# rhasspy/piper

Hardware: AMD Instinct MI355X
Metric: audio samples/sec (higher is better)
Workload: dtype f32; 1 GPU; BASELINE configs[1]: medium VITS voice (22050 Hz), 1 utterance(s) x 128 phoneme ids per step per GPU, scales 0.667/1.0/0.8; step = inferSeconds span: host ids in (pe_upload) + pe_run, engine draws both noise sites + int16 PCM to host (pe_fetch); parallelism=utterance-parallel x1, one process per GPU, RCCL weight broadcast

## Files before the change

piper_amd/csrc/engine.h:

```cpp
#pragma once
#include <cstdint>
#include <deque>
#include <list>
#include <map>
#include <string>
#include <unordered_map>
#include <vector>

#include "pe_rt.h"
#include "engine_buffers.h"
#include "kernels/params.h"
#include "policy.h"
#include "weights.h"

namespace pe {

struct PackedConv {
  float* wp = nullptr;
  float* wp16 = nullptr;
  float* wpb = nullptr;
  const float* wunscale = nullptr;
  float* wpg4 = nullptr;
  float* bias = nullptr;
  int rows = 0;
// ... 224 lines not shown
  const float* pack_ffn2(const WeightSet& ws, const std::string& wname);
  DevBuf<float> ffn_parts_;
  bool stage_a_ffn_fused() const;
  float* stage_a_enc_out() const;
  const float* w4_of(const float* w16) const { auto it = w4_of_.find(w16); return it == w4_of_.end() ? nullptr : it->second; }
  float* dp_proj16_ = nullptr;
  float* dp_pre16_ = nullptr;
  float* projpre4_ = nullptr; float* projpre_bias_ = nullptr; int projpre_split_ = 0;
  void colchain(const struct ColP& p, int B, int Lmax, double flops);
  bool conv1x1_col4(const float* w16, const float* bias, int rows, View in, View out, const int* lens, int B, int Lmax,
                    double flops, const float* bias2 = nullptr, long bias2_bs = 0, const float* w4direct = nullptr, int kin = 192,
                    long max_cols = 0);
  const float* pack4_conv_pad192(const WeightSet& ws, const std::string& wname, int in_rev, int out_rev);
  struct Rcl;
  void pack_gate4pre(const WeightSet& ws, const std::string& prefix, bool odd, Rcl& r);
  void gate_pre(const Rcl& r, View x0, View out, const int* lens, int Lmax, double cols, const float* b2);
  struct LnSecond { const float* w4 = nullptr; int split = 0; View out2{nullptr, 0, 0}; const float* bias2 = nullptr; long bias2_bs = 0; };
  void lngemm(View y, const float* g, const float* b, View x, const float* w16, const float* bias, int rows, View out,
              int T, double flops, const float* parts = nullptr, int nparts = 0, const float* pbias = nullptr,
              const LnSecond* second = nullptr);
  bool proj_pre_stacked() const;
  float* pack16_conv(const WeightSet& ws, const std::string& wname, int in_rev, int out_rev);
  int xcc_of_[64] = {0};
  int xcd_period_ = 0;
  void probe_xcds();
  static size_t col4_smem() { return ((size_t)4 * 196 + 4 * 192 * 4 + 32 + 64 * 4) * sizeof(float); }
  void issue_stage_a();
  void issue_stage_b();
  void issue_flow();
  void issue_window();
// ... 43 lines not shown
    float* proj16 = nullptr;
  };
  std::vector<CFlow> cflows_;
  float ea_m0_ = 0, ea_es0_ = 1;
  float *ea_dev_m_ = nullptr, *ea_dev_logs_ = nullptr;
 public:
  void arena_ready();
 private:
  struct Rcl {
    PackedConv pre, post;
    float *pre16 = nullptr, *post16 = nullptr;
    const float* pre4pad = nullptr;
    std::vector<PackedConv> in, rs;
    std::vector<const float*> rs4;
    const float* gpre4 = nullptr; const float* gpre_bias = nullptr; const float* gpre_tapb = nullptr;
    int in_off, out_off;
  };
  std::vector<Rcl> rcls_;
  PackedConv dec_pre_;
  struct UpStage {
    PackedConv up;
    int rate, ch;
    std::vector<std::vector<PackedConv>> rb;
    float* last_bias_sum = nullptr;
    struct HostConv { std::vector<float> w; int co = 0, ci = 0, k = 0, dil = 1; const float* bias = nullptr; };
    std::vector<std::vector<HostConv>> rb_host;
    void* mrf_phases = nullptr; float* mrf_w = nullptr;
    float* mrf_wsplit = nullptr; float* mrf_unscale = nullptr; int mrf_wsplit_floats = 0;
    int mrf_wfloats = 0, mrf_cp = 0, mrf_hx = 0;
    std::vector<struct MrfPhase> mrf_ph;
// ... 243 lines not shown
```

piper_amd/csrc/engine_issue.cpp:

```cpp
#include "engine_internal.h"

namespace pe {

bool Engine::stage_a_ffn_fused() const {
  double tsum = 0;
  for (int b = 0; b < B_; ++b) tsum += tlens_h_[b];
  const bool chain_q = pol_.chain16(tsum, false, H_, 96);
  bool f = pol_.ffn && chain_q && pol_.chain4((long)B_ * Tg_) && ffn_parts_ && (long)B_ * rup(Tg_, 4) <= LaunchPolicy::ffn_max_cols &&
           FC_ % 48 == 0 && FC_ / 48 <= 16 && w4_of(enc_proj16_);
  for (auto& e : enc_) f = f && e.f1p && e.f2p && w4_of(e.qkv16);
  return f;
}
bool Engine::proj_pre_stacked() const {
  double tsum = 0;
  for (int b = 0; b < B_; ++b) tsum += tlens_h_[b];
  return pol_.stack_pre && projpre4_ && projpre_split_ == enc_proj_.rows && dp_pre_.rows == 192 && H_ == 192 &&
         pol_.chain16(tsum, false, H_, 96) && pol_.chain4((long)B_ * Tg_);
}
float* Engine::stage_a_enc_out() const { return (stage_a_ffn_fused() && (enc_.size() & 1)) ? y_ : x_; }

void Engine::issue_stage_a() {
  const int B = B_, Ts = Ts_, T = Tg_;
  const long bsH = (long)H_ * Ts;
  auto V = [&](float* p, int ch) { return View{p, (long)ch * Ts, Ts}; };
// ... 279 lines not shown
    PE_LAUNCH_KB("regulate_kernel", 4.0 * (2.0 * C_ * cols_ids_ + 3.0 * C_ * fsum), launch::regulate(dim3((Fmax + 255) / 256, (C_ + 3) / 4, B), stream_, rp));
    if (zp_keep_)
      PE_HIP(hipMemcpyAsync(zp_keep_, zp_, (size_t)B * C_ * Fs * sizeof(float), hipMemcpyDeviceToDevice, stream_));
  }
  auto VF = [&](float* p, int ch) { return View{p, (long)ch * Fs, Fs}; };
  const View fh = VF(fh_, H_), facts = VF(facts_, H_), fskip = VF(fskip_, H_);
  const int half = C_ / 2;
  const bool chain = pol_.chain16(fsum, true, H_, half);
  auto rs_front_of = [&](size_t ri, bool front = true) {
    const Rcl& r = rcls_[ri];
    const int nl = (int)r.in.size();
    return chain && nl >= 1 && r.rs4[nl - 1] && r.rs[nl - 1].rows == H_ && H_ == 192 && half == 96 &&
           (front ? pol_.chain_rs_front((long)B * Fmax) : pol_.chain4_frames((long)B * Fmax)) && w4_of(r.post16) &&
           (ri + 1 >= rcls_.size() || (rcls_[ri + 1].pre.rows <= 192 && w4_of(rcls_[ri + 1].pre16)));
  };
  auto compose_pre_of = [&](size_t ri) {
    if (ri >= rcls_.size() || !pol_.compose_pre() || !rs_front_of(ri, false)) return false;
    const Rcl& r = rcls_[ri];
    return r.in.size() >= 2 && r.gpre4 && r.rs4[0] && r.rs[0].rows == 2 * H_ && w4_of(r.pre16) && r.pre.rows == H_ &&
           plan_conv(r.in[0], Fmax, EPI_GATE, stage_tiled_).form == CONV_GATE12;
  };
  for (size_t ri = 0; ri < rcls_.size(); ++ri) {
    Rcl& r = rcls_[ri];
    const View x0{zp_ + (long)r.in_off * Fs, (long)C_ * Fs, Fs};
    const View x1{zp_ + (long)r.out_off * Fs, (long)C_ * Fs, Fs};
    const bool compose_pre = compose_pre_of(ri);
    if (!(chain && ri > 0) && !compose_pre) {
      if (!(chain && r.pre4pad && conv1x1_col4(nullptr, r.pre.bias, r.pre.rows, x0, fh, lens_b_, B, Fmax, 2.0 * fsum * r.pre.macs_per_col,
                                               nullptr, 0, r.pre4pad, half, LaunchPolicy::col4_max_frames)))
        conv(r.pre, x0, fh, lens_b_, 1, Fmax, EPI_STORE);
    }
    const int nl = (int)r.in.size();
    const bool rs_front = rs_front_of(ri);
    for (int i = 0; i < nl; ++i) {
      const float* b2 = nspk_ > 1 ? cond_ + cond_off_wn_[ri] + (long)i * 2 * H_ : nullptr;
      if (compose_pre && i == 0) gate_pre(r, x0, facts, lens_b_, Fmax, fsum, b2);
      else conv(r.in[i], fh, facts, lens_b_, 1, Fmax, EPI_GATE, {.bias2 = b2, .bias2_bs = cond_bs_});
      if (rs_front && i == nl - 1) {
        fl += 2.0 * fsum * (r.in[i].macs_per_col + r.rs[i].macs_per_col);
        continue;
      }
      if (r.rs4[i] && pol_.chain4_frames((long)B * Fmax) && H_ == 192 && r.rs[i].rows <= 2 * H_) {
        ColP cp{};
        cp.in1 = facts.p; cp.in1_bs = facts.bs; cp.in1_cs = facts.cs; cp.K1 = H_;
        cp.w1 = r.rs4[i]; cp.b1 = r.rs[i].bias; cp.rows1 = r.rs[i].rows;
        cp.mode = 2; cp.first = i == 0 ? 1 : 0;
        cp.xcd = xcd_period_;
        cp.x1 = fh.p; cp.x1_bs = fh.bs; cp.x1_cs = fh.cs;
        cp.out = fskip.p; cp.out_bs = fskip.bs; cp.out_cs = fskip.cs;
        cp.lens = lens_b_;
        const bool hpre = compose_pre && i == 0;
        if (hpre) {
          cp.in0 = x0.p; cp.in0_bs = x0.bs; cp.in0_cs = x0.cs;
          cp.w2 = w4_of(r.pre16); cp.b2 = r.pre.bias; cp.rows2 = H_;
        }
        const int kh4 = kbegin(prof_level_ >= 2 ? krow("colchain4_kernel<false>") : 0,
                               2.0 * fsum * (r.rs[i].macs_per_col + (hpre ? r.pre.macs_per_col : 0)),
                               4.0 * (fsum * (H_ + 2.0 * cp.rows1) + (double)cp.rows1 * H_ + (hpre ? half * (fsum + H_) : 0)));
        launch::colchain4(dim3((Fmax + 3) / 4, B, (cp.rows1 + 191) / 192), col4_smem() + (hpre ? 4 * (96 + 4) * sizeof(float) : 0), stream_, cp);
        kend(kh4);
      } else {
        conv(r.rs[i], facts, fh, lens_b_, 1, Fmax, EPI_WNRS, {.out2 = fskip, .mode = i == 0 ? 1 : 0});
      }
      fl += 2.0 * fsum * (r.in[i].macs_per_col + r.rs[i].macs_per_col);
    }
    if (chain) {
      ColP cp{};
      cp.in1 = fskip.p; cp.in1_bs = fskip.bs; cp.in1_cs = fskip.cs; cp.K1 = H_;
      cp.w1 = r.post16; cp.b1 = r.post.bias; cp.rows1 = half;
      cp.mode = 1;
      cp.x1 = x1.p; cp.x1_bs = x1.bs; cp.x1_cs = x1.cs;
      if (ri + 1 < rcls_.size() && !compose_pre_of(ri + 1)) {
        const Rcl& nx = rcls_[ri + 1];
        if (nx.in_off != r.out_off) throw std::runtime_error("coupling layers do not alternate halves");
        cp.w2 = nx.pre16; cp.b2 = nx.pre.bias; cp.rows2 = H_;
        cp.out2 = fh.p; cp.o2_bs = fh.bs; cp.o2_cs = fh.cs;
      }
      cp.lens = lens_b_;
      if (rs_front) {
        cp.in0 = facts.p; cp.in0_bs = facts.bs; cp.in0_cs = facts.cs;
        cp.w0 = r.rs4[nl - 1]; cp.b0 = r.rs[nl - 1].bias; cp.first = nl == 1 ? 1 : 0;
      }
      colchain(cp, B, Fmax, 2.0 * fsum * (r.post.macs_per_col + (cp.w2 ? rcls_[ri + 1].pre.macs_per_col : 0) +
                                          (rs_front ? r.rs[nl - 1].macs_per_col : 0)));
    } else {
      conv(r.post, fskip, x1, lens_b_, 1, Fmax, EPI_SUBFROM);
    }
    fl += 2.0 * fsum * (r.pre.macs_per_col + r.post.macs_per_col);
  }
  prof_end(2, fl);

}

void Engine::issue_stage_b() {
  issue_flow();
  double fsum = 0;
  for (int b = 0; b < B_; ++b) fsum += frames_h_[b];
  issue_decoder(zp_, lens_b_, Fg_, fsum, false);
}
// ... 193 lines not shown
```

piper_amd/csrc/engine_launch.cpp:

```cpp
#include "engine_internal.h"

namespace pe {


static int tile_cfg_of(int cfg) { return cfg == CFG_C ? CFG_C : CFG_S; }
static int slab_halo(int xhalo) { return xhalo <= 64 ? 64 : 128; }
static size_t tile_smem(int nbuf, int BN, int halo) { return (size_t)nbuf * KC * ((BN + halo + 63) / 64 * 64) * sizeof(float); }
static size_t splitk_smem(int nw, int MT, int xw) { return std::max<size_t>((size_t)nw * KC * xw, (size_t)nw * MT * 16 * 64) * sizeof(float); }

ConvPlan Engine::plan_conv(const PackedConv& pc, int Lmax, int epi, bool stage_tiled) const {
  ConvPlan pl;
  const bool convt = epi == EPI_CONVT;
  const int ncols = pl.ncols = convt ? Lmax + 1 : Lmax;
  const int xhalo = (pc.ntaps - 1) * pc.dil, units = pc.nchunks * pc.ntaps;
  pl.blocks = tile_workgroups(CFG_BM[pc.cfg], CFG_BN[pc.cfg], ncols, pc.mtiles, B_);
  pl.halo = slab_halo(xhalo);
  const bool to_splitk = !stage_tiled && pol_.splitk(pl.blocks, xhalo, pc.Cin);
  const bool direct = pol_.one_tap_direct(pc.gate, convt, pc.ntaps, pc.Cin);
  pl.group_splitk = !stage_tiled && !convt && pol_.groupable(pc.gate, pc.up != 0, pl.blocks, xhalo, pc.Cin);
  pl.group_tiled = !pc.gate && pc.up == 0 && !convt && !to_splitk && !(matrix_bf3_ && pc.wpb) && !direct && xhalo <= 128;
  pl.group_cfg = tile_cfg_of(pc.cfg);
  if (to_splitk && epi == EPI_GATE &&
      pol_.gate_12col(pc.gate, pc.wpg4 != nullptr && pc.Cin == 192, pc.ntaps, pc.dil, tile_workgroups(32, 12, ncols, pc.split / 32, B_))) {
    pl.form = CONV_GATE12;
// ... 490 lines not shown
  cp.mode = 3;
  cp.xcd = xcd_period_;
  cp.res = bias2; cp.res_bs = bias2_bs;
  cp.out = out.p; cp.out_bs = out.bs; cp.out_cs = out.cs;
  cp.lens = lens;
  if (kt_on_ && out.p == qkv_ && rows == 3 * H_) { cp.kT = kT_; cp.vQ = vQ_; cp.kt_bs = (long)Ts_ * H_; kt_valid_ = true; }
  const double cols = lens == d_tlens_ ? cols_ids_ : cols_frames_;
  const int kh4 = kbegin(prof_level_ >= 2 ? krow("colchain4_kernel<false>") : 0, flops, 4.0 * (cols * (kin + rows) + (double)rows * kin));
  launch::colchain4(dim3((Lmax + 3) / 4, B, (rows + 191) / 192), col4_smem(), stream_, cp);
  kend(kh4);
  return true;
}

void Engine::colchain(const ColP& p, int B, int Lmax, double flops) {
  const double cols = p.lens == d_tlens_ ? cols_ids_ : cols_frames_;
  const double kbytes = 4.0 * (cols * (p.K1 + 2.0 * p.rows1 + (p.w2 ? p.rows2 : 0)) + (double)p.rows1 * p.K1 +
                               (p.w2 ? (double)p.rows2 * p.rows1 : 0.0));
  if ((p.mode == 1 ? pol_.chain4_frames((long)B * Lmax) : pol_.chain4((long)B * Lmax)) && p.K1 == 192 && (p.mode == 0 ? p.rows1 == 192 : (p.rows1 == 96 && (!p.w2 || p.rows2 <= 192)))) {
    const float* w1 = w4_of(p.w1);
    const float* w2 = p.w2 ? w4_of(p.w2) : nullptr;
    if (w1 && (!p.w2 || w2)) {
      ColP q = p;
      q.w1 = w1; q.w2 = w2;
      q.xcd = xcd_period_;
      const double kb0 = q.w0 ? 4.0 * (cols * 192.0 + 192.0 * 192.0) : 0.0;
      const int kh4 = kbegin(prof_level_ >= 2 ? krow(q.w0 ? "colchain4_kernel<true>" : "colchain4_kernel<false>") : 0, flops, kbytes + kb0);
      launch::colchain4(dim3((Lmax + 3) / 4, B), col4_smem(), stream_, q);
      kend(kh4);
      return;
    }
  }
  if (p.w0) throw std::runtime_error("internal: a res/skip conv in front of a chain that does not take the 4-column form");
  const int kh = kbegin(prof_level_ >= 2 ? krow("colchain_kernel<6>") : 0, flops, kbytes);
  const size_t smem = ((size_t)2 * 6 * 32 * 16 + 16 * 16) * sizeof(float);
  launch::colchain(dim3((Lmax + 15) / 16, B), smem, stream_, p);
  kend(kh);
}

int Engine::kbegin(int row, double flops, double bytes) {
  if (prof_level_ < 2) return -1;
  hipEvent_t a, b;
  if (ev_pool_.size() >= 2) {
    a = ev_pool_.back(); ev_pool_.pop_back();
    b = ev_pool_.back(); ev_pool_.pop_back();
  } else {
    PE_HIP(hipEventCreate(&a));
    PE_HIP(hipEventCreate(&b));
// ... 45 lines not shown
```

piper_amd/csrc/engine_pack.cpp:

```cpp
#include "engine_internal.h"
#include <cmath>

namespace pe {


float* Engine::dev_alloc(size_t nfloats, const float* src) {
  arena_off_ = (arena_off_ + 255) / 256 * 256;
  const size_t bytes = std::max<size_t>(nfloats, 1) * sizeof(float);
  if (arena_off_ + bytes > arena_bytes_) throw std::runtime_error("internal: packed weights exceed the arena bound");
  float* d = reinterpret_cast<float*>(arena_ + arena_off_);
  arena_off_ += bytes;
  if (src && nfloats && !skeleton_) PE_HIP(hipMemcpy(d, src, nfloats * sizeof(float), hipMemcpyHostToDevice));
  weight_bytes_ += nfloats * sizeof(float);
  return d;
}
float* Engine::dev_copy(const std::vector<float>& v) { return dev_alloc(v.size(), v.data()); }

float* Engine::dev_tensor(const WeightSet& ws, const std::string& name) {
  const HostTensor& t = ws.get(name);
  return dev_alloc((size_t)t.numel(), t.data.empty() ? nullptr : t.data.data());
}

size_t Engine::arena_bound(const WeightSet& ws) {
  size_t n = 0;
// ... 339 lines not shown
          bk += a * bp[c];
        }
        for (int i = 0; i < Ci; ++i)
          G[((((size_t)g * nt + k) * (Ci / 4) + i / 4) * 64 + lane) * 4 + (i & 3)] = (float)acc[i];
        tapb[(size_t)k * R + row] = (float)bk;
        bs += bk;
      }
      bsum[row] = (float)bs;
    }
  }
  r.gpre4 = dev_alloc(n4, skeleton_ ? nullptr : G.data());
  r.gpre_bias = dev_alloc((size_t)R, skeleton_ ? nullptr : bsum.data());
  r.gpre_tapb = dev_alloc((size_t)6 * R, skeleton_ ? nullptr : tapb.data());
}

DdsW Engine::load_dds(const WeightSet& ws, const std::string& p) {
  DdsW d;
  for (int i = 0; i < arch_[A_DDSLAYERS]; ++i) {
    const std::string s = std::to_string(i);
    d.dw_w.push_back(dev_tensor(ws, p + ".convs_sep." + s + ".weight"));
    d.dw_b.push_back(dev_tensor(ws, p + ".convs_sep." + s + ".bias"));
    d.c1x1.push_back(pack_conv(ws, p + ".convs_1x1." + s + ".weight", p + ".convs_1x1." + s + ".bias", 1, -1,
                               false, 0, 0));
    {
      const HostTensor& w1 = ws.get(p + ".convs_1x1." + s + ".weight");
      d.w16.push_back(pack16(w1.data, (int)w1.dims[0], (int)w1.dims[1]));
    }
    d.g1.push_back(dev_tensor(ws, p + ".norms_1." + s + ".gamma"));
    d.b1.push_back(dev_tensor(ws, p + ".norms_1." + s + ".beta"));
    d.g2.push_back(dev_tensor(ws, p + ".norms_2." + s + ".gamma"));
// ... 122 lines not shown
        r.in.push_back(pack_conv(ws, p + ".enc.in_layers." + s + ".weight", p + ".enc.in_layers." + s + ".bias",
                                 1, -1, true, 0, 0));
        r.rs.push_back(pack_conv(ws, p + ".enc.res_skip_layers." + s + ".weight",
                                 p + ".enc.res_skip_layers." + s + ".bias", 1, -1, false, 0, 0));
        {
          const HostTensor& wrs = ws.get(p + ".enc.res_skip_layers." + s + ".weight");
          r.rs4.push_back(wrs.dims.size() == 3 && wrs.dims[2] == 1 ? pack4(wrs.data, (int)wrs.dims[0], (int)wrs.dims[1]) : nullptr);
        }
        (void)wnk;
      }
      r.post = pack_conv(ws, p + ".post.weight", p + ".post.bias", 1, -1, false, 0, odd);
      r.pre16 = pack16_conv(ws, p + ".pre.weight", odd, 0);
      if (H_ == 192 && rcls_.empty()) r.pre4pad = pack4_conv_pad192(ws, p + ".pre.weight", odd, 0);
      r.post16 = pack16_conv(ws, p + ".post.weight", 0, odd);
      if (wnl >= 2) pack_gate4pre(ws, p, odd, r);
      rcls_.push_back(r);
      if (gin_) {
        const HostTensor& cw = ws.get(p + ".enc.cond_layer.weight");
        cond_wn_.push_back(CondW{dev_tensor(ws, p + ".enc.cond_layer.weight"), dev_tensor(ws, p + ".enc.cond_layer.bias"),
                                 (int)cw.dims[0]});
      }
    }
    if (flips & 1) throw std::runtime_error("odd number of flow layers is not supported");
  }

  dec_pre_ = pack_conv(ws, "dec.conv_pre.weight", "dec.conv_pre.bias", 1, -1, false, 0, 0);
  {
    const int nk = arch_[A_NRB], nd = arch_[A_NDIL];
    int ch = U_;
    for (int i = 0; i < arch_[A_NUPS]; ++i) {
// ... 224 lines not shown
```

piper_amd/csrc/kernels/col4.h:

```cpp
#pragma once
#include "dds.h"

namespace pe {

__device__ __forceinline__ int c4_tile(int bx, int nx, int P) { return pe_xcd_tile(bx, nx, P); }

constexpr int FFN_MAXS = 16;
constexpr int C4_H = 192, C4_NT = C4_H / 64;
template <int K>
struct Col4W {
  static constexpr int NQ = K / 16;
  static constexpr int KS = K + 4;
  f32x4 w[C4_NT][K / 16];
};
template <int K>
__device__ __forceinline__ void col_gemm4_fetch(Col4W<K>& W, const float* wp4, int nt, int wv, int lane) {
  constexpr int NQ = Col4W<K>::NQ, tile_floats = (K / 4) * 256;
#pragma unroll
  for (int m = 0; m < C4_NT; ++m) {
    const bool live = PE_UNIFORM(m < nt);
    const pe_rowsrc ws = pe_make_row_u(wp4 + (long)(live ? m : 0) * tile_floats, live ? tile_floats : 0);
#pragma unroll
    for (int q = 0; q < NQ; ++q) W.w[m][q] = pe_row_load4(ws, ((NQ * wv + q) * 64 + lane) * 4);
  }
// ... 59 lines not shown
}


template <bool FRONT>
__global__ __launch_bounds__(256) void colchain4_kernel(const int* lens, const float* in1, long in1_bs, int nx, int xcd, int mode,
                                                        int in1_cs, int K1r, int rows1, int first, int out_cs, ColP p) {
  PE_KTRACE(3);
  constexpr int NC = 4, NVT = 3, K1 = C4_H, K2 = C4_H / 2, KS1 = Col4W<K1>::KS, KS2 = Col4W<K2>::KS;
  PE_DYN_SMEM(float, sm);
  if constexpr (!FRONT) PE_STAMP(3, 0);
  p.lens = lens; p.xcd = xcd; p.mode = mode; p.in1 = in1; p.in1_bs = in1_bs; p.in1_cs = in1_cs; p.K1 = K1r; p.rows1 = rows1;
  p.first = first; p.out_cs = out_cs;
  const int b = blockIdx.y;
  int L = PE_UNIFORM(lens[b]);
  if constexpr (FRONT) PE_ENTRY_BATCH(L, p.res, p.res_bs, p.res_cs, p.gamma, p.beta, p.out, p.out_bs, p.x1, p.x1_bs, p.x1_cs, p.b1, p.w1,
                                      p.in0, p.in0_bs, p.in0_cs, p.w0, p.b0);
  else PE_ENTRY_BATCH(L, p.res, p.res_bs, p.res_cs, p.gamma, p.beta, p.out, p.out_bs, p.x1, p.x1_bs, p.x1_cs, p.b1, p.w1,
                      p.in0, p.in0_bs, p.in0_cs, p.w2, p.b2, p.kT, p.kt_bs, p.vQ);
  const int t0 = c4_tile(blockIdx.x, nx, p.xcd) * NC;
  if (t0 >= L) return;
  if constexpr (!FRONT) PE_STAMP(3, 1);
  float* YT = sm;
  float* P = YT + NC * KS1;
  float* red = P + 4 * C4_H * NC;
  const int tid = threadIdx.x, col = tid & 3, rl = tid >> 2, wv = PE_UNIFORM(tid >> 6), lane = tid & 63;
  const int t = t0 + col;
  const bool ok = t < L;
  const int part = p.mode >= 2 ? (int)blockIdx.z : 0, row0 = part * C4_H;
  const int rows_here = p.rows1 - row0 < C4_H ? p.rows1 - row0 : C4_H;
  Col4W<K1> gw0;
  Col4W<K1> gw;
  auto fetch_gw = [&]() { col_gemm4_fetch<K1>(gw, p.w1 + (long)part * C4_NT * (K1 / 4) * 256, (rows_here + 63) / 64, wv, lane); };
  const bool skip_part = p.mode == 2 && (p.rows1 <= C4_H || part == 1);
  const bool pre_part = !FRONT && p.mode == 2 && p.w2 && !skip_part;
  float* YTP = P + 4 * C4_H * NC + 32 + 64 * 4;
  Col4W<K2> gw2;
  float sk[NVT];
  if constexpr (FRONT) {
    const pe_rowsrc a0 = pe_make_row(p.in0 + (long)b * p.in0_bs, K1 * p.in0_cs);
    const pe_rowsrc s0 = pe_make_row(p.in1 + (long)b * p.in1_bs, p.first ? 0 : K1 * p.in1_cs);
    const pe_rowsrc b0d = pe_make_row(p.b0 ? p.b0 : p.w0, p.b0 ? K1 : 0);
    float av[NVT], b0v[NVT];
#pragma unroll
    for (int k = 0; k < NVT; ++k) {
      const int c = rl + 64 * k;
      av[k] = pe_row_load(a0, ok ? c * p.in0_cs + t : -1);
      sk[k] = pe_row_load(s0, ok ? c * p.in1_cs + t : -1);
      b0v[k] = pe_row_load(b0d, c);
    }
    PE_SCHED_FENCE();
    col_gemm4_fetch<K1>(gw0, p.w0, C4_NT, wv, lane);
// ... 34 lines not shown
    PE_SCHED_FENCE();
    if constexpr (!FRONT) fetch_gw();
    if (pre_part) col_gemm4_fetch<K2>(gw2, p.w2, C4_NT, wv, lane);
    if constexpr (!FRONT) PE_STAMP(3, 2);
#pragma unroll
    for (int k = 0; k < NVT; ++k) YT[col * KS1 + rl + 64 * k] = xin[k];
    if constexpr (!FRONT)
      if (pre_part) {
        YTP[col * KS2 + rl] = x0v[0];
        if (rl < K2 - 64) YTP[col * KS2 + rl + 64] = x0v[1];
      }
  }
  __syncthreads();
  if (pre_part) col_gemm4_run2<K1, K2>(gw, YT, gw2, YTP, P, wv, lane);
  else col_gemm4_run<K1>(gw, YT, P, wv, lane);
  const bool second = p.mode == 1 && p.w2;
  if (second) col_gemm4_fetch<K2>(gw2, p.w2, (p.rows2 + 63) / 64, wv, lane);
  __syncthreads();

  if (p.mode >= 2) {
    if (!ok) return;
    float* tp = (skip_part || p.mode == 3) ? p.out + (long)b * p.out_bs + (p.mode == 3 ? (long)row0 * p.out_cs : 0) : p.x1 + (long)b * p.x1_bs;
    const int tcs = (skip_part || p.mode == 3) ? p.out_cs : p.x1_cs;
#pragma unroll
    for (int k = 0; k < NVT; ++k) {
      const int c = rl + 64 * k;
      if (c < rows_here) {
        const float val = (col_gemm4_get(P, c, col) + b1v[k]) + ov[k];
        tp[(long)c * tcs + t] = val;
        if (p.mode == 3 && p.kT && part == 1) p.kT[(long)b * p.kt_bs + ((long)(c >> 2) * p.out_cs + t) * 4 + (c & 3)] = val;
        if (p.mode == 3 && p.vQ && part == 2) p.vQ[(long)b * p.kt_bs + ((long)(t >> 2) * C4_H + c) * 4 + (t & 3)] = val;
// ... 17 lines not shown
    float q = 0.f;
#pragma unroll
    for (int k = 0; k < NVT; ++k)
      if (rl + 64 * k < H) { const float d = v[k] - mean; q = fmaf(d, d, q); }
    const float rstd = 1.f / sqrtf(col_sum(q) / (float)H + 1e-5f);
    if (!ok) return;
    float* ob = p.out + (long)b * p.out_bs;
#pragma unroll
    for (int k = 0; k < NVT; ++k) {
      const int c = rl + 64 * k;
      if (c < H) ob[(long)c * p.out_cs + t] = (v[k] - mean) * rstd * gg[k] + bb[k];
    }
    return;
  }

  {
    float* xb = p.x1 + (long)b * p.x1_bs;
    float* YT2 = YT;
    const pe_rowsrc b2d = pe_make_row(second ? p.b2 : p.w1, (second && p.b2) ? p.rows2 : 0);
    float b2v[NVT];
#pragma unroll
    for (int k = 0; k < NVT; ++k) b2v[k] = pe_row_load(b2d, rl + 64 * k);
#pragma unroll
    for (int k = 0; k < NVT; ++k) {
      const int c = rl + 64 * k;
      if (c < K2) {
        const float xn = (ok && c < p.rows1) ? ov[k] - (col_gemm4_get(P, c, col) + b1v[k]) : 0.f;
        if (ok && c < p.rows1) xb[(long)c * p.x1_cs + t] = xn;
        YT2[col * KS2 + c] = xn;
      }
    }
    if (!second) return;
    __syncthreads();
    col_gemm4_run<K2>(gw2, YT2, P, wv, lane);
    __syncthreads();
    if (!ok) return;
    float* o2 = p.out2 + (long)b * p.o2_bs;
#pragma unroll
    for (int k = 0; k < NVT; ++k) {
      const int c = rl + 64 * k;
      if (c < p.rows2) o2[(long)c * p.o2_cs + t] = col_gemm4_get(P, c, col) + b2v[k];
    }
  }
}

__global__ __launch_bounds__(256) void lngemm4_kernel(const int* lens, int nx, int xcd, const float* in, long in_bs, int in_cs,
                                                      int rows, const float* parts, int nparts, LnGemmP p) {
  PE_KTRACE(7);
  constexpr int NC = 4, NVT = 3, H = C4_H, KS = Col4W<H>::KS;
  PE_DYN_SMEM(float, sm);
  p.lens = lens; p.xcd = xcd; p.in = in; p.in_bs = in_bs; p.in_cs = in_cs; p.rows = rows; p.parts = parts; p.nparts = nparts;
  const int b = blockIdx.y;
  int L = PE_UNIFORM(lens[b]);
  PE_ENTRY_BATCH(L, p.gamma, p.beta, p.bias, p.pbias, p.p_bs, p.w16);
  const int t0 = c4_tile(blockIdx.x, nx, p.xcd) * NC;
  if (t0 >= L) return;
  float* YT = sm;
  float* P = YT + NC * KS;
// ... 87 lines not shown
```

piper_amd/csrc/policy.cpp:

```cpp
#include "policy.h"

#include <cerrno>
#include <cstdio>
#include <cstdlib>
#include <cstring>
#include <mutex>
#include <stdexcept>
#include <string>

namespace pe {

static const LaunchPolicy::Knob kKnobs[] = {
    {"PIPER_HIP_MRF", &LaunchPolicy::mrf, 0, 2, "fused MRF stage kernel: 0 off (conv by conv), 1 by the measured policy (ResBlock2 stages always; ResBlock1 stages on 32 channels up to PIPER_HIP_MRF_MAXF frames per call), 2 wherever it applies"},
    {"PIPER_HIP_MRF_MAXF", &LaunchPolicy::mrf_maxf, 0, 1L << 40, "batch frames up to which a 32-channel ResBlock1 stage runs in the fused kernel (mode 1)"},
    {"PIPER_HIP_MRF_OU", &LaunchPolicy::mrf_ou, 0, 4, "force the output units per wave of mrf_kernel (1..4) instead of the cost model; ignored when the width does not fit"},
    {"PIPER_HIP_MRF_TAIL", &LaunchPolicy::mrf_tail, 0, 1, "generator tail inside the last stage's mrf_kernel (0: separate conv_post_kernel)"},
    {"PIPER_HIP_MRF_SPLIT", &LaunchPolicy::mrf_split, 0, 1, "matrix modes bf16x3 / f16x3: the fused MRF stage kernel on the 16-bit matrix pipe with split operands (mrf_split_kernel) wherever a fused stage applies; 0 = the f32 fused kernel below PIPER_HIP_BF3_MINF frames, conv by conv on the 16-bit pipe above"},
    {"PIPER_HIP_BF3_MINF", &LaunchPolicy::bf3_minf, 0, 1L << 40, "split matrix modes without a fused 16-bit stage kernel (bf16x6, or PIPER_HIP_MRF_SPLIT=0): batch frames from which the <= 64-channel MRF stages run conv by conv on the 16-bit pipe"},
    {"PIPER_HIP_SPLITK_MAX", &LaunchPolicy::splitk_max, 0, 1L << 40, "tile-workgroup count below which a conv goes to the split-K kernels (0: always the tiled kernel)"},
    {"PIPER_HIP_SPLITK16", &LaunchPolicy::splitk16, 0, 3, "16-column split-K form: 0 off, 1 gate convs, 2 + long-K plain convs, 3 everywhere"},
    {"PIPER_HIP_WIDE_SPLITK", &LaunchPolicy::wide_splitk, 0, 2, "12-wave split-K: 0 off, 1 WN gate conv, 2 always"},
    {"PIPER_HIP_TPB", &LaunchPolicy::tpb, 0, 64, "tiled kernel: column tiles walked by one workgroup (0 = 1)"},
    {"PIPER_HIP_GROUP_MRF", &LaunchPolicy::group_mrf, 0, 2, "sibling resblock convs of a wider small stage as grouped launches (one-utterance calls): 0 off, 2 without the K-concatenated last step"},
    {"PIPER_HIP_GROUP_MAXB", &LaunchPolicy::group_maxb, 0, 1L << 40, "64 x 64 tiles of one conv of a stage below which the grouped sibling launches of a single utterance take the split-K kernels (the tiled grouped launches from there on)"},
// ... 6 lines not shown
    {"PIPER_HIP_ATTN4", &LaunchPolicy::attn4, 0, 2, "attention + conv_o + norm_layers_1 on 4-query workgroups (attn4_kernel) in place of attno_kernel: 0 off, 1 for calls whose longest utterance has up to PIPER_HIP_ATTN4_MAXC ids, 2 wherever attno_kernel applies"},
    {"PIPER_HIP_ATTN4_MAXC", &LaunchPolicy::attn4_maxc, 0, 1L << 40, "ids of the longest utterance of a call up to which attention runs on 4-query workgroups"},
    {"PIPER_HIP_FUSE_DP", &LaunchPolicy::fuse_dp, 0, 1, "ConvFlow.pre / proj / spline fused into the DDSConv layer launches"},
    {"PIPER_HIP_SPEC", &LaunchPolicy::spec, 0, 1, "speculative stage-B sizing / whole utterance as one graph for <= 4 utterances per call"},
    {"PIPER_HIP_SPEC_EXPECT", &LaunchPolicy::spec_expect, 0, 1, "speculative graphs planned for the expected frame counts (0: for the bucket capacity)"},
    {"PIPER_HIP_PCM_ZC", &LaunchPolicy::pcm_zc, 0, 1, "PCM written straight into pinned host memory by pcm16_kernel (0: one copy per utterance behind the graph)"},
    {"PIPER_HIP_IDS_ZC", &LaunchPolicy::ids_zc, 0, 1, "phoneme ids, lengths and speaker ids read straight from the pinned host block by embed_kernel, up to 65536 padded ids per call (0: one host-to-device copy in front of the graph)"},
    {"PIPER_HIP_NO_GRAPH", &LaunchPolicy::no_graph, 0, 1, "launch kernels directly instead of replaying hipGraphs"},
    {"PIPER_HIP_GRAPHS", &LaunchPolicy::graphs, 1, 4096, "hipGraphs kept per engine (least recently used evicted one at a time)"},
    {"PIPER_HIP_CONVT_VEC", &LaunchPolicy::convt_vec, 0, 1, "polyphase up-conv: a lane's four accumulator rows leave as one 16-byte store (stride a multiple of 4) or two 8-byte stores (stride 2) of consecutive output samples; 0: one 4-byte store per phase"},
    {"PIPER_HIP_XCD", &LaunchPolicy::xcd, -1, 32, "XCDs the dispatch round-robins over, for the XCD-aware tile orders (-1 = probed at engine creation, 0 = tiles in workgroup order)"},
    {"PIPER_HIP_XCD_FFN", &LaunchPolicy::xcd_ffn, 0, 1, "ffn_kernel deals (column tile, slice) to the XCDs slice-major, so an XCD's L2 holds two slices' weights instead of all sixteen (0: blockIdx order)"},
    {"PIPER_HIP_STACK_PRE", &LaunchPolicy::stack_pre, 0, 1, "small calls of the 192-channel voices: enc_p.proj and dp.pre (both read the last LayerNorm's output) as one lngemm4_kernel launch over the stacked matrix (0: two launches)"},
    {"PIPER_HIP_CHAIN_RS", &LaunchPolicy::chain_rs, 0, 1, "small calls of the 192-channel voices: the last WN layer's res/skip conv (skip rows only) in front of the coupling layer's post + pre chain launch, colchain4_kernel<true> (0: a launch of its own)"},
    {"PIPER_HIP_GATE4", &LaunchPolicy::gate4, 0, 2, "short calls: the WN gate conv over 192 channels on 64-row x 12-column workgroups with the 4x4x1 MFMA (gate4_kernel) up to 640 workgroups: 0 off (16-column split-K form), 2 wherever the split-K route applies"},
    {"PIPER_HIP_WN_COMPOSE", &LaunchPolicy::wn_compose, 0, 3, "short calls of the 192-channel voices, where the coupling chain runs on colchain4_kernel and the gate conv on gate4_kernel: 1x1 convs of a coupling layer composed into their neighbours when the weights are packed: 0 off, 1 every composition that is built, 2 only pre into the first gate conv (gate4pre_kernel over the 96 channels of x0; the coupling layer's pre launch and the chain's pre GEMM go, the first res/skip launch also writes the hidden state's pre term), 3 only post into the skip convs (not built: the route of 0)"},
    {"PIPER_HIP_GATE_HALF", &LaunchPolicy::gate_half, 0, 1, "short one-utterance calls (up to 128 whole-group workgroups): the WN gate conv on half a 32-channel group per workgroup, six waves with the whole K range in flight, twice the workgroups (0: whole groups on twelve waves)"},
    {"PIPER_HIP_CONV1X1", &LaunchPolicy::conv1x1, 0, 1, "batched one-tap convs (q/k/v, WN res/skip, coupling pre/post, proj) through conv1x1_kernel, B operand straight from global memory (0: the tiled kernel)"},
    {"PIPER_HIP_WS_BUDGET_MB", &LaunchPolicy::ws_budget_mb, 0, 1048576, "MiB of device memory the workspace of one pipeline half may take (0: a third of the device's memory): capacities grow only inside it, a call that does not fit by itself is an error"},
    {"PIPER_HIP_ATTN_LONG", &LaunchPolicy::attn_long, 0, 1, "attention score slabs in global memory (attn_long_kernel) at every length, also in place of attno_kernel (tests): by default only utterances whose 32 x T slab does not fit LDS (more than ~830 ids) take that form"},
    {"PIPER_HIP_PROF_SITES", &LaunchPolicy::prof_sites, 0, 1, "level-2 profile rows of the tiled conv kernel per conv shape (tuning aid)"},
    {"PIPER_HIP_DEBUG_KEEP", &LaunchPolicy::debug_keep, 0, 1, "test hook: keep z_p for pe_debug_tensor"},
    {"PIPER_HIP_DEBUG_POISON", &LaunchPolicy::debug_poison, 0, 1, "test hook: activation workspaces are filled with NaN bit patterns when allocated (no kernel may read what the call did not write)"},
};

const LaunchPolicy::Knob* LaunchPolicy::knobs(int* n) {
  if (n) *n = (int)(sizeof(kKnobs) / sizeof(kKnobs[0]));
  return kKnobs;
}

void LaunchPolicy::read_env() {
// ... 45 lines not shown
```

piper_amd/csrc/policy.h:

```cpp
#pragma once
#include <cstddef>

namespace pe {

struct LaunchPolicy {
  long mrf = 1;
  long mrf_maxf = 1100;
  long mrf_ou = 0;
  long mrf_tail = 1;
  long mrf_split = 1;
  long bf3_minf = 1100;
  long splitk_max = 96;
  long splitk16 = 2;
  long wide_splitk = 1;
  long tpb = 0;
  long group_mrf = 1;
  long group_maxb = 160;
  long group_tiled = 1;
  long colchain = 1;
  long col4 = 1;
  long col4_maxc = 1024;
  long ffn = 1;
  long attno = 1;
  long attn4 = 1;
// ... 52 lines not shown
    return gate_half && gate && nchunks == 6 && ntaps <= 5 && 2 * workgroups_whole <= 256;
  }
  static constexpr long gate4_max_workgroups = 640;
  bool gate_12col(bool gate, bool packed4, int ntaps, int dil, long workgroups) const {
    return gate4 && gate && packed4 && ntaps <= 5 && dil == 1 && (gate4 == 2 || workgroups <= gate4_max_workgroups);
  }
  int tiles_per_workgroup() const { return tpb > 0 ? (int)tpb : 1; }
  bool chain16(double cols, bool frames, int k1, int half) const {
    return colchain && k1 == 192 && half == 96 && (colchain == 2 || cols <= (double)(frames ? colchain_max_frames : colchain_max_ids));
  }
  bool chain4(long cols, long limit = 0) const { return col4 && (col4 == 2 || cols <= (limit ? limit : col4_maxc)); }
  bool attn4_ids(long longest_utterance) const { return attn4 == 2 || (attn4 == 1 && longest_utterance <= attn4_maxc); }
  bool chain4_frames(long cols) const { return chain4(cols, col4_max_frames); }
  bool chain_rs_front(long cols) const { return chain_rs && chain4_frames(cols); }
  bool compose_pre() const { return wn_compose == 1 || wn_compose == 2; }
  bool mrf_build(int channels) const { return mrf != 0 && channels <= 64 && channels % 4 == 0; }
  bool mrf_stage(bool built, bool resblock1, int padded_channels, double frames, bool matrix_bf3, bool split_fused = false) const {
    if (mrf && built && split_fused) return mrf == 2 || !resblock1 || padded_channels == 32;
    return mrf && built && !(matrix_bf3 && mrf != 2 && frames >= (double)bf3_minf) &&
           (mrf == 2 || !resblock1 || (padded_channels == 32 && frames <= (double)mrf_maxf));
  }
  bool group_stage(int B, int nk, long blocks64, bool buffers_fit) const {
    return group_mrf && B == 1 && nk >= 2 && nk <= 3 && blocks64 < group_max_blocks64 && blocks64 < group_maxb && buffers_fit;
  }
  bool stage_all_tiled(int B, int nk, long blocks64) const {
    return group_mrf && group_tiled && B == 1 && nk >= 2 && nk <= 3 && blocks64 >= group_maxb;
  }
  bool group_sum() const { return group_mrf != 2; }
  bool group_stage_tiled(int nk, long tile_blocks, bool buffers_fit) const {
    return group_tiled && nk >= 2 && nk <= 3 && tile_blocks <= group_tiled_max_blocks && buffers_fit;
// ... 7 lines not shown
```

Measured before the change: 124.8 million samples/s.

## Compose coupling post 1x1 conv into WN skip convs and drop post GEMM

Precomputes post·skip weight products on the host so each WN res/skip layer writes the 96-row post contribution directly into the skip sum. The coupling chain launch then skips its 192->96 post GEMM through a new no-main path in colchain4_kernel. This removes one GEMM per coupling layer and shrinks the skip output from 192 to 96 rows. The cost is a new kernel branch and extra packed weights. The route only runs when wn_compose is 1 or 4, and the default value is not shown.

```diff
diff --git a/piper_amd/csrc/engine.h b/piper_amd/csrc/engine.h
--- a/piper_amd/csrc/engine.h
+++ b/piper_amd/csrc/engine.h
@@ -262,6 +262,7 @@
   const float* pack4_conv_pad192(const WeightSet& ws, const std::string& wname, int in_rev, int out_rev);
   struct Rcl;
   void pack_gate4pre(const WeightSet& ws, const std::string& prefix, bool odd, Rcl& r);
+  void pack_post4(const WeightSet& ws, const std::string& prefix, bool odd, Rcl& r);
   void gate_pre(const Rcl& r, View x0, View out, const int* lens, int Lmax, double cols, const float* b2);
   struct LnSecond { const float* w4 = nullptr; int split = 0; View out2{nullptr, 0, 0}; const float* bias2 = nullptr; long bias2_bs = 0; };
   void lngemm(View y, const float* g, const float* b, View x, const float* w16, const float* bias, int rows, View out,
@@ -335,6 +336,7 @@
     std::vector<PackedConv> in, rs;
     std::vector<const float*> rs4;
     const float* gpre4 = nullptr; const float* gpre_bias = nullptr; const float* gpre_tapb = nullptr;
+    std::vector<const float*> rsp4, rsp_bias;
     int in_off, out_off;
   };
   std::vector<Rcl> rcls_;
diff --git a/piper_amd/csrc/engine_issue.cpp b/piper_amd/csrc/engine_issue.cpp
--- a/piper_amd/csrc/engine_issue.cpp
+++ b/piper_amd/csrc/engine_issue.cpp
@@ -317,11 +317,20 @@
            (front ? pol_.chain_rs_front((long)B * Fmax) : pol_.chain4_frames((long)B * Fmax)) && w4_of(r.post16) &&
            (ri + 1 >= rcls_.size() || (rcls_[ri + 1].pre.rows <= 192 && w4_of(rcls_[ri + 1].pre16)));
   };
-  auto compose_pre_of = [&](size_t ri) {
-    if (ri >= rcls_.size() || !pol_.compose_pre() || !rs_front_of(ri, false)) return false;
+  auto compose_route_of = [&](size_t ri) {
+    if (ri >= rcls_.size() || !rs_front_of(ri, false)) return false;
     const Rcl& r = rcls_[ri];
     return r.in.size() >= 2 && r.gpre4 && r.rs4[0] && r.rs[0].rows == 2 * H_ && w4_of(r.pre16) && r.pre.rows == H_ &&
            plan_conv(r.in[0], Fmax, EPI_GATE, stage_tiled_).form == CONV_GATE12;
+  };
+  auto compose_pre_of = [&](size_t ri) { return pol_.compose_pre() && compose_route_of(ri); };
+  auto compose_post_of = [&](size_t ri) {
+    if (!pol_.compose_post() || !compose_route_of(ri)) return false;
+    const Rcl& r = rcls_[ri];
+    if (r.rsp4.size() != r.in.size()) return false;
+    for (size_t j = 0; j < r.rsp4.size(); ++j)
+      if (!r.rsp4[j] || !r.rsp_bias[j]) return false;
+    return true;
   };
   for (size_t ri = 0; ri < rcls_.size(); ++ri) {
     Rcl& r = rcls_[ri];
@@ -334,7 +343,7 @@
         conv(r.pre, x0, fh, lens_b_, 1, Fmax, EPI_STORE);
     }
     const int nl = (int)r.in.size();
-    const bool rs_front = rs_front_of(ri);
+    const bool rs_front = rs_front_of(ri), compose_post = compose_post_of(ri);
     for (int i = 0; i < nl; ++i) {
       const float* b2 = nspk_ > 1 ? cond_ + cond_off_wn_[ri] + (long)i * 2 * H_ : nullptr;
       if (compose_pre && i == 0) gate_pre(r, x0, facts, lens_b_, Fmax, fsum, b2);
@@ -347,6 +356,9 @@
         ColP cp{};
         cp.in1 = facts.p; cp.in1_bs = facts.bs; cp.in1_cs = facts.cs; cp.K1 = H_;
         cp.w1 = r.rs4[i]; cp.b1 = r.rs[i].bias; cp.rows1 = r.rs[i].rows;
+        if (compose_post) {
+          cp.w1 = r.rsp4[i]; cp.b1 = r.rsp_bias[i]; cp.rows1 = r.rs[i].rows - H_ + half;
+        }
         cp.mode = 2; cp.first = i == 0 ? 1 : 0;
         cp.xcd = xcd_period_;
         cp.x1 = fh.p; cp.x1_bs = fh.bs; cp.x1_cs = fh.cs;
@@ -358,7 +370,7 @@
           cp.w2 = w4_of(r.pre16); cp.b2 = r.pre.bias; cp.rows2 = H_;
         }
         const int kh4 = kbegin(prof_level_ >= 2 ? krow("colchain4_kernel<false>") : 0,
-                               2.0 * fsum * (r.rs[i].macs_per_col + (hpre ? r.pre.macs_per_col : 0)),
+                               2.0 * fsum * ((double)cp.rows1 * H_ + (hpre ? r.pre.macs_per_col : 0)),
                                4.0 * (fsum * (H_ + 2.0 * cp.rows1) + (double)cp.rows1 * H_ + (hpre ? half * (fsum + H_) : 0)));
         launch::colchain4(dim3((Fmax + 3) / 4, B, (cp.rows1 + 191) / 192), col4_smem() + (hpre ? 4 * (96 + 4) * sizeof(float) : 0), stream_, cp);
         kend(kh4);
@@ -384,8 +396,12 @@
         cp.in0 = facts.p; cp.in0_bs = facts.bs; cp.in0_cs = facts.cs;
         cp.w0 = r.rs4[nl - 1]; cp.b0 = r.rs[nl - 1].bias; cp.first = nl == 1 ? 1 : 0;
       }
-      colchain(cp, B, Fmax, 2.0 * fsum * (r.post.macs_per_col + (cp.w2 ? rcls_[ri + 1].pre.macs_per_col : 0) +
-                                          (rs_front ? r.rs[nl - 1].macs_per_col : 0)));
+      if (compose_post) {
+        cp.K1 = half; cp.w1 = nullptr; cp.b1 = nullptr;
+        if (rs_front) { cp.w0 = r.rsp4[nl - 1]; cp.b0 = r.rsp_bias[nl - 1]; }
+      }
+      colchain(cp, B, Fmax, 2.0 * fsum * ((compose_post ? 0 : r.post.macs_per_col) + (cp.w2 ? rcls_[ri + 1].pre.macs_per_col : 0) +
+                                          (rs_front ? (compose_post ? (double)half * H_ : r.rs[nl - 1].macs_per_col) : 0)));
     } else {
       conv(r.post, fskip, x1, lens_b_, 1, Fmax, EPI_SUBFROM);
     }
diff --git a/piper_amd/csrc/engine_launch.cpp b/piper_amd/csrc/engine_launch.cpp
--- a/piper_amd/csrc/engine_launch.cpp
+++ b/piper_amd/csrc/engine_launch.cpp
@@ -528,23 +528,23 @@
 
 void Engine::colchain(const ColP& p, int B, int Lmax, double flops) {
   const double cols = p.lens == d_tlens_ ? cols_ids_ : cols_frames_;
-  const double kbytes = 4.0 * (cols * (p.K1 + 2.0 * p.rows1 + (p.w2 ? p.rows2 : 0)) + (double)p.rows1 * p.K1 +
+  const double kbytes = 4.0 * (cols * (p.K1 + 2.0 * p.rows1 + (p.w2 ? p.rows2 : 0)) + (p.w1 ? (double)p.rows1 * p.K1 : 0.0) +
                                (p.w2 ? (double)p.rows2 * p.rows1 : 0.0));
-  if ((p.mode == 1 ? pol_.chain4_frames((long)B * Lmax) : pol_.chain4((long)B * Lmax)) && p.K1 == 192 && (p.mode == 0 ? p.rows1 == 192 : (p.rows1 == 96 && (!p.w2 || p.rows2 <= 192)))) {
-    const float* w1 = w4_of(p.w1);
+  if ((p.mode == 1 ? pol_.chain4_frames((long)B * Lmax) : pol_.chain4((long)B * Lmax)) && p.K1 == (p.w1 ? 192 : 96) && (p.mode == 0 ? p.w1 && p.rows1 == 192 : (p.rows1 == 96 && (!p.w2 || p.rows2 <= 192)))) {
+    const float* w1 = p.w1 ? w4_of(p.w1) : nullptr;
     const float* w2 = p.w2 ? w4_of(p.w2) : nullptr;
-    if (w1 && (!p.w2 || w2)) {
+    if ((w1 || !p.w1) && (!p.w2 || w2)) {
       ColP q = p;
       q.w1 = w1; q.w2 = w2;
       q.xcd = xcd_period_;
-      const double kb0 = q.w0 ? 4.0 * (cols * 192.0 + 192.0 * 192.0) : 0.0;
+      const double kb0 = q.w0 ? 4.0 * (cols * 192.0 + (q.w1 ? 192.0 : 96.0) * 192.0) : 0.0;
       const int kh4 = kbegin(prof_level_ >= 2 ? krow(q.w0 ? "colchain4_kernel<true>" : "colchain4_kernel<false>") : 0, flops, kbytes + kb0);
       launch::colchain4(dim3((Lmax + 3) / 4, B), col4_smem(), stream_, q);
       kend(kh4);
       return;
     }
   }
-  if (p.w0) throw std::runtime_error("internal: a res/skip conv in front of a chain that does not take the 4-column form");
+  if (p.w0 || !p.w1) throw std::runtime_error("internal: a res/skip conv in front of a chain that does not take the 4-column form");
   const int kh = kbegin(prof_level_ >= 2 ? krow("colchain_kernel<6>") : 0, flops, kbytes);
   const size_t smem = ((size_t)2 * 6 * 32 * 16 + 16 * 16) * sizeof(float);
   launch::colchain(dim3((Lmax + 15) / 16, B), smem, stream_, p);
diff --git a/piper_amd/csrc/engine_pack.cpp b/piper_amd/csrc/engine_pack.cpp
--- a/piper_amd/csrc/engine_pack.cpp
+++ b/piper_amd/csrc/engine_pack.cpp
@@ -377,6 +377,46 @@
   r.gpre_tapb = dev_alloc((size_t)6 * R, skeleton_ ? nullptr : tapb.data());
 }
 
+void Engine::pack_post4(const WeightSet& ws, const std::string& prefix, bool odd, Rcl& r) {
+  const HostTensor& wpo = ws.get(prefix + ".post.weight");
+  const int nl = (int)r.in.size(), H = 192, half = 96;
+  if (H_ != H || C_ / 2 != half || nl < 1 || wpo.dims.size() != 3 || wpo.dims[2] != 1 || (int)wpo.dims[0] != half || (int)wpo.dims[1] != H) return;
+  for (int j = 0; j < nl; ++j) {
+    const HostTensor& w = ws.get(prefix + ".enc.res_skip_layers." + std::to_string(j) + ".weight");
+    if (!r.rs4[j] || w.dims.size() != 3 || w.dims[2] != 1 || (int)w.dims[1] != H || (int)w.dims[0] != (j < nl - 1 ? 2 * H : H)) return;
+  }
+  const std::string bpn = prefix + ".post.bias";
+  std::vector<double> acc(H);
+  for (int j = 0; j < nl; ++j) {
+    const bool last = j == nl - 1;
+    const int res = last ? 0 : H, rows = res + half;
+    const std::string rsn = prefix + ".enc.res_skip_layers." + std::to_string(j);
+    std::vector<float> W(skeleton_ ? 0 : (size_t)rows * H), B(skeleton_ ? 0 : rows, 0.f);
+    if (!skeleton_) {
+      const HostTensor& w = ws.get(rsn + ".weight");
+      const float* bs = ws.has(rsn + ".bias") ? ws.get(rsn + ".bias").data.data() : nullptr;
+      const float* bpo = ws.has(bpn) ? ws.get(bpn).data.data() : nullptr;
+      std::copy(w.data.begin(), w.data.begin() + (size_t)res * H, W.begin());
+      if (bs) std::copy(bs, bs + res, B.begin());
+      for (int o = 0; o < half; ++o) {
+        const float* pr = &wpo.data[(size_t)(odd ? half - 1 - o : o) * H];
+        std::fill(acc.begin(), acc.end(), 0.0);
+        double c = (j == 0 && bpo) ? (double)bpo[odd ? half - 1 - o : o] : 0.0;
+        for (int s = 0; s < H; ++s) {
+          const double a = pr[s];
+          const float* sr = &w.data[(size_t)(res + s) * H];
+          for (int i = 0; i < H; ++i) acc[i] += a * sr[i];
+          if (bs) c += a * bs[res + s];
+        }
+        for (int i = 0; i < H; ++i) W[(size_t)(res + o) * H + i] = (float)acc[i];
+        B[res + o] = (float)c;
+      }
+    }
+    r.rsp4.push_back(pack4(W, rows, H));
+    r.rsp_bias.push_back(dev_alloc((size_t)rows, skeleton_ ? nullptr : B.data()));
+  }
+}
+
 DdsW Engine::load_dds(const WeightSet& ws, const std::string& p) {
   DdsW d;
   for (int i = 0; i < arch_[A_DDSLAYERS]; ++i) {
@@ -529,6 +569,7 @@
       if (H_ == 192 && rcls_.empty()) r.pre4pad = pack4_conv_pad192(ws, p + ".pre.weight", odd, 0);
       r.post16 = pack16_conv(ws, p + ".post.weight", 0, odd);
       if (wnl >= 2) pack_gate4pre(ws, p, odd, r);
+      pack_post4(ws, p, odd, r);
       rcls_.push_back(r);
       if (gin_) {
         const HostTensor& cw = ws.get(p + ".enc.cond_layer.weight");
diff --git a/piper_amd/csrc/kernels/col4.h b/piper_amd/csrc/kernels/col4.h
--- a/piper_amd/csrc/kernels/col4.h
+++ b/piper_amd/csrc/kernels/col4.h
@@ -97,7 +97,7 @@
   const int b = blockIdx.y;
   int L = PE_UNIFORM(lens[b]);
   if constexpr (FRONT) PE_ENTRY_BATCH(L, p.res, p.res_bs, p.res_cs, p.gamma, p.beta, p.out, p.out_bs, p.x1, p.x1_bs, p.x1_cs, p.b1, p.w1,
-                                      p.in0, p.in0_bs, p.in0_cs, p.w0, p.b0);
+                                      p.in0, p.in0_bs, p.in0_cs, p.w0, p.b0, p.w2, p.b2, p.rows2, p.out2, p.o2_bs, p.o2_cs);
   else PE_ENTRY_BATCH(L, p.res, p.res_bs, p.res_cs, p.gamma, p.beta, p.out, p.out_bs, p.x1, p.x1_bs, p.x1_cs, p.b1, p.w1,
                       p.in0, p.in0_bs, p.in0_cs, p.w2, p.b2, p.kT, p.kt_bs, p.vQ);
   const int t0 = c4_tile(blockIdx.x, nx, p.xcd) * NC;
@@ -111,6 +111,7 @@
   const bool ok = t < L;
   const int part = p.mode >= 2 ? (int)blockIdx.z : 0, row0 = part * C4_H;
   const int rows_here = p.rows1 - row0 < C4_H ? p.rows1 - row0 : C4_H;
+  const bool nomain = p.mode == 1 && !p.w1;
   Col4W<K1> gw0;
   Col4W<K1> gw;
   auto fetch_gw = [&]() { col_gemm4_fetch<K1>(gw, p.w1 + (long)part * C4_NT * (K1 / 4) * 256, (rows_here + 63) / 64, wv, lane); };
@@ -118,6 +119,76 @@
   const bool pre_part = !FRONT && p.mode == 2 && p.w2 && !skip_part;
   float* YTP = P + 4 * C4_H * NC + 32 + 64 * 4;
   Col4W<K2> gw2;
+  const bool second = p.mode == 1 && p.w2;
+  auto chain_tail = [&](auto m_of, const float* ovv) {
+    float* xb = p.x1 + (long)b * p.x1_bs;
+    float* YT2 = YT;
+    const pe_rowsrc b2d = pe_make_row(second ? p.b2 : p.w1, (second && p.b2) ? p.rows2 : 0);
+    float b2v[NVT];
+#pragma unroll
+    for (int k = 0; k < NVT; ++k) b2v[k] = pe_row_load(b2d, rl + 64 * k);
+#pragma unroll
+    for (int k = 0; k < NVT; ++k) {
+      const int c = rl + 64 * k;
+      if (c < K2) {
+        const float xn = (ok && c < p.rows1) ? ovv[k] - m_of(k, c) : 0.f;
+        if (ok && c < p.rows1) xb[(long)c * p.x1_cs + t] = xn;
+        YT2[col * KS2 + c] = xn;
+      }
+    }
+    if (!second) return;
+    __syncthreads();
+    col_gemm4_run<K2>(gw2, YT2, P, wv, lane);
+    __syncthreads();
+    if (!ok) return;
+    float* o2 = p.out2 + (long)b * p.o2_bs;
+#pragma unroll
+    for (int k = 0; k < NVT; ++k) {
+      const int c = rl + 64 * k;
+      if (c < p.rows2) o2[(long)c * p.o2_cs + t] = col_gemm4_get(P, c, col) + b2v[k];
+    }
+  };
+  if (nomain) {
+    const pe_rowsrc s0 = pe_make_row(p.in1 + (long)b * p.in1_bs, (FRONT && p.first) ? 0 : K2 * p.in1_cs);
+    const pe_rowsrc x1d = pe_make_row(p.x1 + (long)b * p.x1_bs, K2 * p.x1_cs);
+    float m[NVT], ovn[NVT];
+    m[2] = ovn[2] = 0.f;
+    if constexpr (FRONT) {
+      const pe_rowsrc a0 = pe_make_row(p.in0 + (long)b * p.in0_bs, K1 * p.in0_cs);
+      const pe_rowsrc b0d = pe_make_row(p.b0 ? p.b0 : p.w0, p.b0 ? K2 : 0);
+      float av[NVT], b0v[2];
+#pragma unroll
+      for (int k = 0; k < NVT; ++k) av[k] = pe_row_load(a0, ok ? (rl + 64 * k) * p.in0_cs + t : -1);
+#pragma unroll
+      for (int k = 0; k < 2; ++k) {
+        const int c = rl + 64 * k;
+        m[k] = pe_row_load(s0, (ok && c < K2) ? c * p.in1_cs + t : -1);
+        b0v[k] = pe_row_load(b0d, c);
+        ovn[k] = pe_row_load(x1d, (ok && c < K2) ? c * p.x1_cs + t : -1);
+      }
+      PE_SCHED_FENCE();
+      col_gemm4_fetch<K1>(gw0, p.w0, (K2 + 63) / 64, wv, lane);
+#pragma unroll
+      for (int k = 0; k < NVT; ++k) YT[col * KS1 + rl + 64 * k] = av[k];
+      __syncthreads();
+      if (second) col_gemm4_fetch<K2>(gw2, p.w2, (p.rows2 + 63) / 64, wv, lane);
+      col_gemm4_run<K1>(gw0, YT, P, wv, lane);
+      __syncthreads();
+#pragma unroll
+      for (int k = 0; k < 2; ++k) m[k] = ok ? (col_gemm4_get(P, rl + 64 * k, col) + b0v[k]) + m[k] : 0.f;
+    } else {
+#pragma unroll
+      for (int k = 0; k < 2; ++k) {
+        const int c = rl + 64 * k;
+        m[k] = pe_row_load(s0, (ok && c < K2) ? c * p.in1_cs + t : -1);
+        ovn[k] = pe_row_load(x1d, (ok && c < K2) ? c * p.x1_cs + t : -1);
+      }
+      PE_SCHED_FENCE();
+      if (second) col_gemm4_fetch<K2>(gw2, p.w2, (p.rows2 + 63) / 64, wv, lane);
+    }
+    chain_tail([&](int k, int) { return m[k]; }, ovn);
+    return;
+  }
   float sk[NVT];
   if constexpr (FRONT) {
     const pe_rowsrc a0 = pe_make_row(p.in0 + (long)b * p.in0_bs, K1 * p.in0_cs);
@@ -182,7 +253,6 @@
   __syncthreads();
   if (pre_part) col_gemm4_run2<K1, K2>(gw, YT, gw2, YTP, P, wv, lane);
   else col_gemm4_run<K1>(gw, YT, P, wv, lane);
-  const bool second = p.mode == 1 && p.w2;
   if (second) col_gemm4_fetch<K2>(gw2, p.w2, (p.rows2 + 63) / 64, wv, lane);
   __syncthreads();
 
@@ -230,34 +300,7 @@
     return;
   }
 
-  {
-    float* xb = p.x1 + (long)b * p.x1_bs;
-    float* YT2 = YT;
-    const pe_rowsrc b2d = pe_make_row(second ? p.b2 : p.w1, (second && p.b2) ? p.rows2 : 0);
-    float b2v[NVT];
-#pragma unroll
-    for (int k = 0; k < NVT; ++k) b2v[k] = pe_row_load(b2d, rl + 64 * k);
-#pragma unroll
-    for (int k = 0; k < NVT; ++k) {
-      const int c = rl + 64 * k;
-      if (c < K2) {
-        const float xn = (ok && c < p.rows1) ? ov[k] - (col_gemm4_get(P, c, col) + b1v[k]) : 0.f;
-        if (ok && c < p.rows1) xb[(long)c * p.x1_cs + t] = xn;
-        YT2[col * KS2 + c] = xn;
-      }
-    }
-    if (!second) return;
-    __syncthreads();
-    col_gemm4_run<K2>(gw2, YT2, P, wv, lane);
-    __syncthreads();
-    if (!ok) return;
-    float* o2 = p.out2 + (long)b * p.o2_bs;
-#pragma unroll
-    for (int k = 0; k < NVT; ++k) {
-      const int c = rl + 64 * k;
-      if (c < p.rows2) o2[(long)c * p.o2_cs + t] = col_gemm4_get(P, c, col) + b2v[k];
-    }
-  }
+  chain_tail([&](int k, int c) { return col_gemm4_get(P, c, col) + b1v[k]; }, ov);
 }
 
 __global__ __launch_bounds__(256) void lngemm4_kernel(const int* lens, int nx, int xcd, const float* in, long in_bs, int in_cs,
diff --git a/piper_amd/csrc/policy.cpp b/piper_amd/csrc/policy.cpp
--- a/piper_amd/csrc/policy.cpp
+++ b/piper_amd/csrc/policy.cpp
@@ -44,7 +44,7 @@
     {"PIPER_HIP_STACK_PRE", &LaunchPolicy::stack_pre, 0, 1, "small calls of the 192-channel voices: enc_p.proj and dp.pre (both read the last LayerNorm's output) as one lngemm4_kernel launch over the stacked matrix (0: two launches)"},
     {"PIPER_HIP_CHAIN_RS", &LaunchPolicy::chain_rs, 0, 1, "small calls of the 192-channel voices: the last WN layer's res/skip conv (skip rows only) in front of the coupling layer's post + pre chain launch, colchain4_kernel<true> (0: a launch of its own)"},
     {"PIPER_HIP_GATE4", &LaunchPolicy::gate4, 0, 2, "short calls: the WN gate conv over 192 channels on 64-row x 12-column workgroups with the 4x4x1 MFMA (gate4_kernel) up to 640 workgroups: 0 off (16-column split-K form), 2 wherever the split-K route applies"},
-    {"PIPER_HIP_WN_COMPOSE", &LaunchPolicy::wn_compose, 0, 3, "short calls of the 192-channel voices, where the coupling chain runs on colchain4_kernel and the gate conv on gate4_kernel: 1x1 convs of a coupling layer composed into their neighbours when the weights are packed: 0 off, 1 every composition that is built, 2 only pre into the first gate conv (gate4pre_kernel over the 96 channels of x0; the coupling layer's pre launch and the chain's pre GEMM go, the first res/skip launch also writes the hidden state's pre term), 3 only post into the skip convs (not built: the route of 0)"},
+    {"PIPER_HIP_WN_COMPOSE", &LaunchPolicy::wn_compose, 0, 4, "short calls of the 192-channel voices, where the coupling chain runs on colchain4_kernel and the gate conv on gate4_kernel: 1x1 convs of a coupling layer composed into their neighbours when the weights are packed: 0 off, 1 every composition that is built (pre and post), 2 only pre into the first gate conv (gate4pre_kernel over the 96 channels of x0; the coupling layer's pre launch and the chain's pre GEMM go, the first res/skip launch also writes the hidden state's pre term), 3 the route of 0, 4 only post into the skip convs (every WN layer adds post . skip, 96 rows, into the skip sum; the chain launch's post GEMM goes)"},
     {"PIPER_HIP_GATE_HALF", &LaunchPolicy::gate_half, 0, 1, "short one-utterance calls (up to 128 whole-group workgroups): the WN gate conv on half a 32-channel group per workgroup, six waves with the whole K range in flight, twice the workgroups (0: whole groups on twelve waves)"},
     {"PIPER_HIP_CONV1X1", &LaunchPolicy::conv1x1, 0, 1, "batched one-tap convs (q/k/v, WN res/skip, coupling pre/post, proj) through conv1x1_kernel, B operand straight from global memory (0: the tiled kernel)"},
     {"PIPER_HIP_WS_BUDGET_MB", &LaunchPolicy::ws_budget_mb, 0, 1048576, "MiB of device memory the workspace of one pipeline half may take (0: a third of the device's memory): capacities grow only inside it, a call that does not fit by itself is an error"},
diff --git a/piper_amd/csrc/policy.h b/piper_amd/csrc/policy.h
--- a/piper_amd/csrc/policy.h
+++ b/piper_amd/csrc/policy.h
@@ -90,6 +90,7 @@
   bool chain4_frames(long cols) const { return chain4(cols, col4_max_frames); }
   bool chain_rs_front(long cols) const { return chain_rs && chain4_frames(cols); }
   bool compose_pre() const { return wn_compose == 1 || wn_compose == 2; }
+  bool compose_post() const { return wn_compose == 1 || wn_compose == 4; }
   bool mrf_build(int channels) const { return mrf != 0 && channels <= 64 && channels % 4 == 0; }
   bool mrf_stage(bool built, bool resblock1, int padded_channels, double frames, bool matrix_bf3, bool split_fused = false) const {
     if (mrf && built && split_fused) return mrf == 2 || !resblock1 || padded_channels == 32;
```

Result: faster. 126.3 million samples/s, median of 6 (+1.2%).
